# Martinsos/edlib

Measured on NVIDIA H100. Metric: GCUPS, higher is better.
Workload: dtype u32

## Files before the change

edlib_b200/csrc/eb_common.h:

```cpp
#pragma once
#include <stdint.h>

#if defined(__CUDACC__)
#define EB_HD __host__ __device__ __forceinline__
#define EB_D __device__ __forceinline__
#else
#define EB_HD inline
#define EB_D inline
#endif

namespace eb {

struct U2 { uint32_t x, y; };

constexpr int KPOS = 4;

struct Rec {
    int best;
    int cnt;
    int last;
    int rsv;
    int pos[KPOS];
};

constexpr int KPOSW = 12;
struct WinRec {
    int best, cnt, last, rsv;
    int pos[KPOSW];
};

struct Ovf {
    int rec;
    int score;
    int pos;
};

#define K1_RANGE_GAP 256
#define K1_RANGE_SPAN 1024
#define K1_RANGE_MAX 16

enum Mode : int { MODE_NW = 0, MODE_SHW = 1, MODE_HW = 2 };

struct K1Params {
    const uint8_t* tcodes;
    int n;
    const uint8_t* qcodes;
    const uint64_t* qoff;
    const int* qlen;
    const int* readList;
    const int* kInit;
    int numReads;
    int mode;
    int ncodes;
    const uint8_t* eqtab;
    int chunks;
    int chunkLen;
    int halo;
    Rec* recs;
    Ovf* ovf;
    int* ovfCount;
    int ovfCap;
    int prefixLen;
    int rangeMode;
};

struct K1WParams {
    const uint8_t* tcodes;
    const uint8_t* qcodes;
    const uint64_t* qoff;
    const int* qlen;
    const int* readList;
    const int* kInit;
    const int* winStart;
    const int* winLen;
    const int* trackFrom;
    int numReads;
    const int* countPtr;
    int checkAfter;
    int ncodes;
    const uint8_t* eqtab;
    WinRec* recs;
    Ovf* ovf;
    int* ovfCount;
    int ovfCap;
};

struct LJob {
    uint64_t qOff;
    uint64_t tOff;
    uint64_t matOff;
    int m, n;
    int kInit;
    int trackFrom;
};
struct LParams {
    const LJob* jobs;
    int numJobs;
    const uint8_t* qcodes;
    const uint8_t* tcodes;
    int ncodes;
    const uint8_t* eqtab;
    Rec* recs;
    U2* mat;
    int matStep;
};

enum WFlags : int {
    WF_QREV = 1,
    WF_TREV = 2,
    WF_SLIDE = 4,
    WF_STORE = 8,
    WF_STOPCOL = 16,
};

struct WJob {
    uint64_t qOff;
    uint64_t tOff;
    uint64_t peqOff;
    uint64_t auxOff;
    uint64_t hbufOff;
    int m, n;
    int nWp;
    int mode;
    int flags;
    int kInit;
    int dhi;
    int stopCol;
    int rec;
    int trackFrom;
};

struct WParams {
    const WJob* jobs;
    int numJobs;
    const uint8_t* qcodes;
    const uint8_t* tcodes;
    const uint32_t* peq;
// ... 250 lines not shown
```

edlib_b200/csrc/eb_core.h:

```cpp
#pragma once
#include "eb_common.h"

#if defined(__CUDA_ARCH__)
#define EB_UNROLL _Pragma("unroll")
#else
#define EB_UNROLL
#endif

namespace eb {


EB_HD uint32_t funnel_l1(uint32_t lo, uint32_t hi) {
#if defined(__CUDA_ARCH__)
    return __funnelshift_l(lo, hi, 1);
#else
    return (hi << 1) | (lo >> 31);
#endif
}

EB_HD int popcount32(uint32_t v) {
#if defined(__CUDA_ARCH__)
    return __popc(v);
#else
    return __builtin_popcount(v);
#endif
}

EB_HD int atomic_add_int(int* p, int v) {
#if defined(__CUDA_ARCH__)
    return atomicAdd(p, v);
#else
    int old = *p;
    *p = old + v;
    return old;
#endif
}

EB_HD void atomic_max_int(int* p, int v) {
#if defined(__CUDA_ARCH__)
    atomicMax(p, v);
#else
    if (v > *p) *p = v;
#endif
}

EB_HD void atomic_or_u32(uint32_t* p, uint32_t v) {
#if defined(__CUDA_ARCH__)
    atomicOr(p, v);
#else
    *p |= v;
#endif
}

template <int NW>
struct AddChain {
    static EB_HD void run(uint32_t (&S)[NW], const uint32_t (&T)[NW], const uint32_t (&P)[NW]) {
        uint32_t carry = 0;
        EB_UNROLL
        for (int w = 0; w < NW; ++w) {
            uint64_t s = (uint64_t)T[w] + P[w] + carry;
            S[w] = (uint32_t)s;
            carry = (uint32_t)(s >> 32);
        }
    }
};
#if defined(__CUDA_ARCH__)
template <>
struct AddChain<1> {
    static EB_HD void run(uint32_t (&S)[1], const uint32_t (&T)[1], const uint32_t (&P)[1]) { S[0] = T[0] + P[0]; }
};
template <>
struct AddChain<2> {
    static EB_HD void run(uint32_t (&S)[2], const uint32_t (&T)[2], const uint32_t (&P)[2]) {
        asm("add.cc.u32 %0, %2, %4;\n\taddc.u32 %1, %3, %5;"
            : "=&r"(S[0]), "=&r"(S[1]) : "r"(T[0]), "r"(T[1]), "r"(P[0]), "r"(P[1]));
    }
};
template <>
struct AddChain<3> {
    static EB_HD void run(uint32_t (&S)[3], const uint32_t (&T)[3], const uint32_t (&P)[3]) {
        asm("add.cc.u32 %0, %3, %6;\n\taddc.cc.u32 %1, %4, %7;\n\taddc.u32 %2, %5, %8;"
            : "=&r"(S[0]), "=&r"(S[1]), "=&r"(S[2])
            : "r"(T[0]), "r"(T[1]), "r"(T[2]), "r"(P[0]), "r"(P[1]), "r"(P[2]));
    }
};
template <>
struct AddChain<4> {
// ... 414 lines not shown
        }
        for (int k = 31; k >= 1; --k) {
            cur += (int)((VN0 >> k) & 1u) - (int)((VP0 >> k) & 1u);
            mn = cur < mn ? cur : mn;
        }
        return mn;
    }

    template <bool TRACK>
    EB_HD void column(int j, uint32_t sym) {
        const int gt = j + g0;
        const int wi = gt >> 5, sh = gt & 31;
        const uint32_t w0 = acc.load_word(sym, wi), w1 = acc.load_word(sym, wi + 1), w2 = acc.load_word(sym, wi + 2);
        const uint32_t Eq0 = funnel_r(w0, w1, sh), Eq1 = funnel_r(w1, w2, sh);
        uint32_t T[2] = {Eq0 & VP0, Eq1 & VP1}, P[2] = {VP0, VP1}, Sm[2];
        AddChain<2>::run(Sm, T, P);
        const uint32_t D00 = ((Sm[0] ^ VP0) | Eq0) | VN0, D01 = ((Sm[1] ^ VP1) | Eq1) | VN1;
        const uint32_t HP0 = VN0 | ~(D00 | VP0), HP1 = VN1 | ~(D01 | VP1);
        const uint32_t HN0 = VP0 & D00, HN1 = VP1 & D01;
        const uint32_t X0 = funnel_r(D00, D01, 1), X1 = D01 >> 1;
        VN0 = X0 & HP0;
        VN1 = X1 & HP1;
        VP0 = HN0 | ~(X0 | HP0);
        VP1 = HN1 | ~(X1 | HP1);
        S += 1 - (int)(HN1 >> 31);
        if (TRACK && j >= lo) {
            constexpr int CAP = (int)(sizeof(rec->pos) / sizeof(rec->pos[0]));
            const int kb = kb0 - j;
            const uint64_t M = kb >= 63 ? 0ull : (~0ull << (kb + 1));
            const int score = S - popcount32(VP0 & (uint32_t)M) - popcount32(VP1 & (uint32_t)(M >> 32)) +
                              popcount32(VN0 & (uint32_t)M) + popcount32(VN1 & (uint32_t)(M >> 32));
            if (score <= best) {
                if (score < best) {
                    best = score;
                    cnt = 0;
                }
                if (cnt < CAP) {
                    rec->pos[cnt] = ws + j;
                } else if (prm.ovfCap > 0) {
                    const int at = atomic_add_int(prm.ovfCount, 1);
                    if (at < prm.ovfCap) {
                        prm.ovf[at].rec = slot;
                        prm.ovf[at].score = score;
                        prm.ovf[at].pos = ws + j;
                    }
                }
                rec->last = ws + j;
                cnt++;
            }
        }
    }
};

template <class WAcc, class RecT>
EB_HD void k1b_sweep(const WAcc& acc, const uint8_t* tsyms, int ws, int m, int off, int c0, int lo, int hi, int t,
                     int checkAfter, int& bestIo, int& cntIo, RecT* rec, const K1WParams& prm, int slot) {
    const int dhi = hi - (m - 1) + t;
    K1Band<WAcc, RecT> b{acc, rec, 0, 0, 0, 0, 0, bestIo, cntIo, off + 64 - dhi, lo, m - 2 + dhi, ws, prm, slot};
    const int firstReal = off + 64 - (c0 + b.g0);
    const uint64_t vp64 = firstReal <= 0 ? ~0ull : (firstReal >= 64 ? 0ull : (~0ull << firstReal));
    b.VP0 = (uint32_t)vp64;
    b.VP1 = (uint32_t)(vp64 >> 32);
    const int bottomRow = c0 - dhi + 63;
    b.S = bottomRow >= 0 ? bottomRow + 1 : 0;
    int j = c0;
    for (; j <= hi && (j & 15); ++j) b.template column<true>(j, tsyms[j]);
    if (j + 15 <= hi) {
        Sym16 v = load_sym16(tsyms + j);
        bool checked = checkAfter < 0 || t == 0;
        for (; j + 15 < lo; j += 16) {
            if (!checked && j >= dhi + checkAfter) {
                checked = true;
                if (b.window_min() > t) return;
            }
            const Sym16 cur = v;
            if (j + 31 <= hi) v = load_sym16(tsyms + j + 16);
            EB_UNROLL
            for (int q = 0; q < 16; ++q) b.template column<false>(j + q, (cur.w[q >> 2] >> (8 * (q & 3))) & 255u);
        }
        for (; j + 15 <= hi; j += 16) {
            const Sym16 cur = v;
            if (j + 31 <= hi) v = load_sym16(tsyms + j + 16);
            EB_UNROLL
            for (int q = 0; q < 16; ++q) b.template column<true>(j + q, (cur.w[q >> 2] >> (8 * (q & 3))) & 255u);
        }
    }
    for (; j <= hi; ++j) b.template column<true>(j, tsyms[j]);
    bestIo = b.best;
    cntIo = b.cnt;
}

template <int NW, class WAcc>
EB_HD void k1w_thread(const K1WParams& p, int slot, WAcc& acc) {
    const int pair = p.readList[slot];
    const int m = p.qlen[pair];
    WinRec* rec = p.recs + slot;
    for (int code = 0; code < p.ncodes; ++code) {
        acc.store_word(code, 0, ~0u);
        acc.store_word(code, 1, ~0u);
        acc.store_word(code, NW + 2, 0u);
        acc.store_word(code, NW + 3, 0u);
    }
    K1View<NW, WAcc> k1acc{acc};
    k1_build_peq<NW>(k1acc, p.qcodes + p.qoff[pair], m, MODE_HW, p.ncodes, p.eqtab);
    const int ws = p.winStart[slot], tf = p.trackFrom[slot], len = p.winLen[slot];
    const int kInit = p.kInit[slot];
    const int t = kInit - 1;
    const int hi = len - 1;
    if (t >= 0 && (hi - tf) + 2 * t + 1 <= 64) {
        const int c0 = tf - (m + t) > 0 ? tf - (m + t) : 0;
        int best = kInit, cnt = 0;
        k1b_sweep(acc, p.tcodes + ws, ws, m, 32 * NW - m, c0, tf, hi, t, p.checkAfter, best, cnt, rec, p, slot);
        rec->best = best;
        rec->cnt = cnt;
        return;
    }
    K1State<NW> st;
    k1_init<NW>(st, m, kInit);
    bool hopeless = false;
    for (int j = 0; j < tf; j += 32) {
        const int cntj = tf - j < 32 ? tf - j : 32;
        k1_columns<NW, false, false>(st, k1acc, PtrSyms{p.tcodes + ws + j}, cntj, ws + j, rec, slot, nullptr, nullptr, 0);
        if (st.up - st.down - (len - (j + cntj)) >= st.best) {
            hopeless = true;
            break;
        }
    }
    if (!hopeless)
        k1_columns<NW, false, true>(st, k1acc, PtrSyms{p.tcodes + ws + tf}, len - tf, ws + tf, rec, slot, p.ovf, p.ovfCount, p.ovfCap);
    rec->best = st.best;
    rec->cnt = st.cnt;
}


EB_HD uint32_t seed_key(const uint8_t* s, int avail, int Lidx, uint32_t sigma) {
    uint32_t key = 0;
    for (int x = 0; x < Lidx; ++x) key = key * sigma + (x < avail ? (uint32_t)s[x] : 0u);
    return key;
}
EB_HD void seed_count_item(const SeedIndexParams& p, int i) {
    atomic_add_int(p.bucketStart + seed_key(p.tcodes + i, p.n - i, p.Lidx, (uint32_t)p.sigma), 1);
}
EB_HD void seed_fill_item(const SeedIndexParams& p, int i) {
    const uint32_t b = seed_key(p.tcodes + i, p.n - i, p.Lidx, (uint32_t)p.sigma);
    p.positions[p.bucketStart[b] + atomic_add_int(p.cursor + b, 1)] = i;
}

template <class F>
EB_HD int seed_windows(const SeedPlanParams& p, const int* E, int c, int m, int t, F&& f) {
    const int bandSlack = 63 - 4 * t;
    int prevHi = -1;
    int nW = 0;
    for (int i = 0; i < c;) {
        const int first = E[i];
        int last = first;
        ++i;
        if (bandSlack >= 0) {
            while (i < c && E[i] - first <= bandSlack) last = E[i++];
        } else {
            while (i < c && E[i] - last <= K1_RANGE_GAP && E[i] - first <= p.spread) last = E[i++];
        }
        int lo = first - t, hi = last + t;
        if (lo <= prevHi) lo = prevHi + 1;
        if (lo < 0) lo = 0;
        if (hi > p.n - 1) hi = p.n - 1;
        if (lo > hi) continue;
        prevHi = hi;
        int ws = lo - (m + t);
        if (ws < 0) ws = 0;
        ws &= ~15;
        f(nW, ws, lo, hi);
        ++nW;
    }
    return nW;
}
EB_HD void seed_window_store(const SeedPlanParams& p, int w, int pair, int t, int ws, int lo, int hi) {
    p.winPair[w] = pair;
    p.winK[w] = t + 1;
    p.winStart[w] = ws;
    p.winLen[w] = hi - ws + 1;
    p.winTf[w] = lo - ws;
}

struct CoopSerial {
// ... 1079 lines not shown
```

edlib_b200/csrc/eb_engine.cpp:

```cpp
#include "eb_engine_internal.h"

#include <sched.h>

namespace eb {

static int env_int(const char* name, int dflt) {
    const char* s = getenv(name);
    return (s && *s) ? atoi(s) : dflt;
}

static std::vector<int> parse_cpulist(const char* path) {
    std::vector<int> cpus;
    FILE* f = fopen(path, "r");
    if (!f) return cpus;
    char buf[4096];
    if (fgets(buf, sizeof(buf), f)) {
        for (char* tok = strtok(buf, ",\n"); tok; tok = strtok(nullptr, ",\n")) {
            int a = 0, b = 0;
            const int got = sscanf(tok, "%d-%d", &a, &b);
            if (got == 1) b = a;
            if (got >= 1)
                for (int c = a; c <= b && c < 4096; ++c) cpus.push_back(c);
        }
    }
// ... 6 lines not shown
    if (cpus.empty()) return;
    cpu_set_t allowed, want;
    CPU_ZERO(&allowed);
    CPU_ZERO(&want);
    if (sched_getaffinity(0, sizeof(allowed), &allowed) != 0) return;
    int n = 0;
    for (int c : cpus)
        if (c < CPU_SETSIZE && CPU_ISSET(c, &allowed)) {
            CPU_SET(c, &want);
            ++n;
        }
    if (n > 0) sched_setaffinity(0, sizeof(want), &want);
}

void host_parallel_ranges(size_t n, size_t grain, const std::function<void(size_t, size_t)>& fn) {
    parallel_ranges(n, grain, [&](size_t lo, size_t hi) { fn(lo, hi); });
}

Engine::Engine(Backend* be) : be_(be) {
    if (env_int("EDLIB_B200_NUMA", 1) == 0) return;
    const int node = be->numa_node();
    if (node < 0) return;
    char path[128];
    snprintf(path, sizeof(path), "/sys/devices/system/node/node%d/cpulist", node);
    std::vector<int> cpus = parse_cpulist(path);
    if (!cpus.empty() && HostPool::worker_cpus().empty()) HostPool::worker_cpus() = cpus;
}

EngineTunables::EngineTunables() {
    k1MinGroup = env_int("EDLIB_B200_K1_MIN_GROUP", k1MinGroup);
    k1MinChunk = env_int("EDLIB_B200_K1_MIN_CHUNK", k1MinChunk);
    ovfCap = env_int("EDLIB_B200_OVF_CAP", ovfCap);
    filterK0 = env_int("EDLIB_B200_FILTER_K0", filterK0);
    filterK1 = env_int("EDLIB_B200_FILTER_K1", filterK1);
    packParallelBytes = (size_t)env_int("EDLIB_B200_PACK_PARALLEL_KB", (int)(packParallelBytes >> 10)) << 10;
    filterSeedK = env_int("EDLIB_B200_FILTER_SEED_K", filterSeedK);
    filterSeedBucket = env_int("EDLIB_B200_FILTER_SEED_BUCKET", filterSeedBucket);
    filterSeedSlack = env_int("EDLIB_B200_FILTER_SEED_SLACK", filterSeedSlack);
    filterMinLevelReads = env_int("EDLIB_B200_FILTER_MIN_LEVEL_READS", filterMinLevelReads);
    tinySweepReads = env_int("EDLIB_B200_TINY_SWEEP_READS", tinySweepReads);
    filterSeedLevels = std::min(SEED_LEVELS, env_int("EDLIB_B200_FILTER_SEED_LEVELS", filterSeedLevels));
    filterMaxWindows = env_int("EDLIB_B200_FILTER_MAX_WINDOWS", filterMaxWindows);
    filterMinLen = env_int("EDLIB_B200_FILTER_MIN_LEN", filterMinLen);
    filterSpread = env_int("EDLIB_B200_FILTER_SPREAD", filterSpread);
    filterMinTarget = env_int("EDLIB_B200_FILTER_MIN_TARGET", filterMinTarget);
    filterSkipRepeats = env_int("EDLIB_B200_FILTER_SKIP_REPEATS", filterSkipRepeats);
    bandKernel = env_int("EDLIB_B200_BAND_KERNEL", bandKernel);
    collapseEqualities = env_int("EDLIB_B200_COLLAPSE_EQUALITIES", collapseEqualities);
    directUpload = env_int("EDLIB_B200_DIRECT_UPLOAD", directUpload);
    streamSlices = std::max(1, env_int("EDLIB_B200_STREAM_SLICES", streamSlices));
    directMinBytes = (size_t)env_int("EDLIB_B200_DIRECT_MIN_KB", (int)(directMinBytes >> 10)) << 10;
    deviceStage = env_int("EDLIB_B200_DEVICE_STAGE", deviceStage);
    windowCheckAfter = env_int("EDLIB_B200_WINDOW_CHECK", windowCheckAfter);
    longHwMinTarget = env_int("EDLIB_B200_LONG_HW_MIN_TARGET", longHwMinTarget);
    longSeedMaxK = env_int("EDLIB_B200_LONG_SEED_MAX_K", longSeedMaxK);
    devSliceReads = std::max(64, env_int("EDLIB_B200_SLICE_READS", devSliceReads));
    streamMinPairs = env_int("EDLIB_B200_STREAM_MIN_PAIRS", streamMinPairs);
    const int sliceMb = env_int("EDLIB_B200_SLICE_MB", 0);
    if (sliceMb > 0) sliceBytes = (size_t)sliceMb << 20;
    if (sliceMb > 0) pathSliceBytes = (size_t)sliceMb << 20;
}

static int code_map(const uint32_t (&present)[8], uint8_t (&map)[256], int other) {
    int ncodes = 0;
    for (int b = 0; b < 256; ++b) ncodes += (present[b >> 5] >> (b & 31)) & 1u;
    int next = 0;
    for (int b = 0; b < 256; ++b) {
        if (present[b >> 5] >> (b & 31) & 1u) map[b] = (uint8_t)next++;
        else map[b] = (uint8_t)(other < 0 ? 0 : std::min(other, 255));
    }
    return ncodes;
}

static int encode_target(Backend* be, uint8_t* raw, int n, TargetCodes& tc) {
    std::vector<MaskItem> items;
    for (int s0 = 0; s0 < n; s0 += 65536) items.push_back(MaskItem{(uint64_t)s0, std::min(65536, n - s0), 0});
    DevBuf<MaskItem> dItems(be, items.size());
    dItems.upload(items.data(), items.size());
    tc.dMask.alloc(be, 8);
    be->zero(tc.dMask.p, 8 * sizeof(uint32_t));
    MaskParams mp;
    memset(&mp, 0, sizeof(mp));
    mp.raw = raw;
    mp.items = dItems.p;
    mp.numItems = (int)items.size();
    mp.masks = tc.dMask.p;
    mp.unionSet = -1;
    be->launch_mask(mp);
    uint32_t present[8];
    be->d2h(present, tc.dMask.p, sizeof(present));
    int distinct = 0;
    for (int b = 0; b < 256; ++b) distinct += (present[b >> 5] >> (b & 31)) & 1u;
    uint8_t map[256];
    code_map(present, map, distinct);
    tc.dMap.alloc(be, 256);
    tc.dMap.upload(map, 256);
    EncodeParams ep{raw, (uint64_t)round_up((size_t)n, 16), tc.dMap.p};
    be->launch_encode(ep);
    tc.ncodes = distinct >= 256 ? 256 : std::max(1, std::min(distinct, 255));
    return tc.ncodes;
}

Prepared* Engine::take_prepared(const BatchInput& in) {
    if (!spare_) spare_ = new Prepared();
    Prepared* p = spare_;
    p->bind(be_);
// ... 1040 lines not shown
```

edlib_b200/csrc/eb_engine.h:

```cpp
#pragma once
#include <stddef.h>
#include <stdint.h>

#include <map>
#include <string>
#include <utility>
#include <vector>

#include "../../include/edlib.h"
#include "eb_common.h"

namespace eb {

struct Backend {
    virtual ~Backend() {}
    virtual void* alloc(size_t bytes) = 0;
    virtual void free(void* p) = 0;
    virtual void* alloc_host(size_t bytes) = 0;
    virtual void free_host(void* p) = 0;
    virtual bool host_pinned(const void* , size_t ) { return false; }
    virtual void h2d(void* dst, const void* src, size_t bytes) = 0;
    virtual void d2h(void* dst, const void* src, size_t bytes) = 0;
    virtual void zero(void* dst, size_t bytes) = 0;
    virtual void d2d(void* dst, const void* src, size_t bytes) = 0;
// ... 12 lines not shown
    virtual int sm_count() = 0;
    virtual void k1_shape(int nw32, int ncodes, int numReads, int* blockThreads, int* residentCtas) = 0;
    virtual void launch_mask(const MaskParams& p) = 0;
    virtual void launch_alpha_len(const uint32_t* masks, const int* qset, const int* tset, int numPairs, int* out) = 0;
    virtual void launch_encode(const EncodeParams& p) = 0;
    virtual void launch_k1(const K1Params& p, int nw32) = 0;
    virtual void launch_k1t(const K1Params& p, int nw32) = 0;
    virtual void launch_k1w(const K1WParams& p, int nw32) = 0;
    virtual void launch_lane(const LParams& p, int nw32, int mode, bool reversed, bool store) = 0;
    virtual void launch_peq(const PeqParams& p) = 0;
    virtual void launch_w(const WParams& p, int R) = 0;
    virtual int band_max_blocks(int ncodes) = 0;
    virtual void launch_band(const WParams& p, int NB, int ncodes) = 0;
    virtual void launch_traceback(const TbParams& p) = 0;
    virtual void launch_res(const ResParams& p) = 0;
    virtual void launch_split(const SplitParams& p) = 0;
    virtual void launch_seed_count(const SeedIndexParams& p) = 0;
    virtual void launch_scan(int* data, int count) = 0;
    virtual void launch_seed_fill(const SeedIndexParams& p) = 0;
    virtual void launch_seed_plan(const SeedPlanParams& p) = 0;
    virtual void launch_win_reduce(const WinReduceParams& p) = 0;
    virtual void launch_fin_count(const FinParams& p) = 0;
    virtual void launch_fin_fill(const FinParams& p) = 0;
    virtual void launch_qalpha(const QAlphaParams& p) = 0;
    virtual void reset_timing() = 0;
    virtual double kernel_ms(const char* nameOrNull) = 0;
    virtual int launches() = 0;
    virtual std::string kernel_report() = 0;
};

struct BatchInput {
    const char* const* queries;
    const int* queryLengths;
    const char* const* targets;
    const int* targetLengths;
    int numPairs;
    EdlibAlignConfig config;
    bool strands = false;
};

struct EngineTunables {
    int k1MinGroup = 32;
    int k1MinChunk = 1024;
    int ovfCap = 1 << 20;
    size_t sliceBytes = 1ull << 30;
    size_t pathSliceBytes = 8ull << 30;
    size_t packParallelBytes = 32u << 20;
    int deviceStage = 1;
    int devSliceReads = 1 << 20;
    int streamSlices = 8;
    int streamMinPairs = 32768;
    int longHwMinTarget = 65536;
    int longSeedMaxK = 1024;
    int windowCheckAfter = 48;
    int filterSeedK = 20;
    int filterSeedBucket = 128;
    int filterSeedLevels = 4;
    int tinySweepReads = 8;
    int filterMinLevelReads = 64;
    int filterSeedSlack = 4;
    int filterK1 = 8;
    int filterK0 = 16;
    int filterMinLen = 96;
    int filterSpread = 1024;
    int filterMaxWindows = 32;
    int filterMinTarget = 65536;
    size_t directMinBytes = 1u << 20;
    int directUpload = 1;
    int collapseEqualities = 1;
    int bandKernel = 1;
    int filterSkipRepeats = 1;
    EngineTunables();
};

struct EngineStats {
    double kernelMs = 0;
    double k1Ms = 0;
    int launches = 0;
    long long h2dBytes = 0, d2hBytes = 0;
    long long k1Cells = 0;
    long long wCells = 0;
    long long filterDecided = 0, filterFallback = 0;
    long long filterWindows = 0;
    std::string kernelReport;
};

struct EngineScratch {
    std::vector<int> best, cnt, posLen, posPool;
    std::vector<long long> posStart;
    int seedWindowsPerRead[SEED_LEVELS] = {0, 0, 0, 0};
    std::vector<int> targetTable;
};

class Prepared;
struct TargetHandle;

class Engine {
public:
    explicit Engine(Backend* be);
    ~Engine();
    int align_batch(const BatchInput& in, EdlibAlignResult* results, unsigned char* strands = nullptr);
    void strands_of(const Prepared* p, unsigned char* strands) const;

    Prepared* prepare(const BatchInput& in);
    void compute(Prepared* p);
    void materialize(Prepared* p, EdlibAlignResult* results, const std::vector<int>* list = nullptr);
    void release(Prepared* p);
// ... 25 lines not shown
```

edlib_b200/csrc/eb_kernels.cu:

```cuda
#include <cuda_runtime.h>
#include <ctype.h>
#include <stdio.h>
#include <sys/syscall.h>
#include <unistd.h>
#include <stdlib.h>
#include <string.h>

#include <algorithm>
#include <mutex>
#include <stdexcept>
#include <string>
#include <vector>

#include "eb_core.h"
#include "eb_dispatch.h"
#include "eb_engine.h"

namespace eb {

#if defined(__CUDA_ARCH__)
#define EB_DEV(expr, fallback) expr
#else
#define EB_DEV(expr, fallback) fallback
#endif
// ... 213 lines not shown
    EB_D void store(int code, int word, uint32_t bits) { w[code * NW + word] = bits; }
    EB_D void or_word(int code, int word, uint32_t bits) { w[code * NW + word] |= bits; }
    EB_D void load(uint32_t code, uint32_t (&Eq)[NW]) const {
#pragma unroll
        for (int i = 0; i < NW; ++i) Eq[i] = w[code * NW + i];
    }
};
template <int NW>
__global__ void __launch_bounds__(32) k1t_kernel(const K1Params p) {
    extern __shared__ __align__(16) unsigned char smem[];
    WarpPeqAcc<NW> acc{reinterpret_cast<uint32_t*>(smem)};
    const int slot = blockIdx.y;
    const int chunk = blockIdx.x * 32 + threadIdx.x;
    if (threadIdx.x == 0) {
        const int pair = p.readList[slot];
        k1_build_peq<NW>(acc, p.qcodes + p.qoff[pair], p.qlen[pair], p.mode, p.ncodes, p.eqtab);
    }
    __syncwarp();
    if (chunk < p.chunks) k1_thread<NW, WarpPeqAcc<NW>, false>(p, slot, chunk, acc);
}

template <int THREADS, int WORDS>
struct SmemWordAcc {
    uint32_t base;
    static constexpr uint32_t wordStride = 4u * THREADS, codeStride = wordStride * WORDS;
    EB_D void store_word(int code, int w, uint32_t bits) {
        asm volatile("st.shared.u32 [%0], %1;" ::"r"(base + (uint32_t)code * codeStride + (uint32_t)w * wordStride), "r"(bits) : "memory");
    }
    EB_D void or_word(int code, int w, uint32_t bits) {
        const uint32_t addr = base + (uint32_t)code * codeStride + (uint32_t)w * wordStride;
        uint32_t v;
        asm volatile("ld.shared.u32 %0, [%1];" : "=r"(v) : "r"(addr) : "memory");
        asm volatile("st.shared.u32 [%0], %1;" ::"r"(addr), "r"(v | bits) : "memory");
    }
    EB_D uint32_t load_word(uint32_t code, int w) const {
        uint32_t v;
        asm volatile("ld.shared.u32 %0, [%1];" : "=r"(v) : "r"(base + code * codeStride + (uint32_t)w * wordStride));
        return v;
    }
};

template <int NW, int THREADS>
__global__ void __launch_bounds__(THREADS) k1w_kernel(const K1WParams p) {
    extern __shared__ __align__(128) unsigned char smem[];
    const int slot = blockIdx.x * THREADS + threadIdx.x;
    int numJobs = p.numReads;
    if (p.countPtr) numJobs = min(numJobs, *p.countPtr);
    if (slot >= numJobs) return;
    SmemWordAcc<THREADS, NW + 4> acc;
    acc.base = smem_u32(smem) + 4u * threadIdx.x;
    k1w_thread<NW>(p, slot, acc);
}

template <int NW, int MODE, bool REV, bool STORE>
__global__ void lane_kernel(const LParams p) {
    extern __shared__ __align__(128) unsigned char smem[];
    const int job = blockIdx.x * blockDim.x + threadIdx.x;
    if (job >= p.numJobs) return;
    SmemPeqAcc<NW> acc;
    acc.codeStride = (uint32_t)blockDim.x * (16u + 4u * SmemPeqAcc<NW>::NWB);
    acc.a0 = smem_u32(smem) + 16u * threadIdx.x;
    acc.b0 = smem_u32(smem) + 16u * blockDim.x + 4u * SmemPeqAcc<NW>::NWB * threadIdx.x;
    lane_job<NW, MODE, REV, STORE>(p, job, acc);
}

constexpr int W_WARPS = 4;

template <int R>
__global__ void __launch_bounds__(W_WARPS * 32) w_kernel(const WParams p) {
    const int job = blockIdx.x * W_WARPS + (threadIdx.x >> 5);
    if (job >= p.numJobs) return;
    w_dispatch<DevWarp, R>(p, job);
}

template <int THREADS, int SLOTS>
struct SmemBandAcc {
    uint32_t base, cur;
    static constexpr uint32_t wordStride = 4u * THREADS, codeStride = wordStride * SLOTS;
    EB_D void set(int code, int slot, uint32_t bits) {
        asm volatile("st.shared.u32 [%0], %1;" ::"r"(base + (uint32_t)code * codeStride + (uint32_t)slot * wordStride), "r"(bits) : "memory");
    }
    EB_D uint32_t get(int code, int slot) const {
        uint32_t v;
        asm volatile("ld.shared.u32 %0, [%1];" : "=r"(v) : "r"(base + (uint32_t)code * codeStride + (uint32_t)slot * wordStride) : "memory");
        return v;
    }
    EB_D void origin(int slot) { cur = base + (uint32_t)slot * wordStride; }
    EB_D uint32_t code_off(uint32_t sym) const { return sym * codeStride; }
    EB_D uint32_t load(uint32_t codeOff, int w) const {
        uint32_t v;
        asm volatile("ld.shared.u32 %0, [%1];" : "=r"(v) : "r"(cur + codeOff + (uint32_t)w * wordStride) : "memory");
        return v;
    }
};
constexpr int BAND_THREADS = 128;
template <int NB>
__global__ void __launch_bounds__(BAND_THREADS) band_kernel(const WParams p, int ncodes) {
    extern __shared__ __align__(128) unsigned char smem[];
    const int job = blockIdx.x * BAND_THREADS + threadIdx.x;
    if (job >= p.numJobs) return;
    SmemBandAcc<BAND_THREADS, 4 * NB + BAND_SLACK> acc;
    acc.base = smem_u32(smem) + 4u * threadIdx.x;
    acc.cur = acc.base;
    band_job<NB>(p, job, acc, ncodes);
}

// ... 465 lines not shown
        size_t smem;
        k1_block(nw, ncodes, numReads, &block, &smem);
        if (shapeCache.empty()) shapeCache.assign(4 * 9 * 1024, 0);
        const int blockClass = block >= 256 ? 3 : block >= 128 ? 2 : block >= 64 ? 1 : 0;
        const int key = (blockClass * 9 + nw) * 1024 + (ncodes < 1024 ? ncodes : 1023);
        if (ncodes < 1023 && shapeCache[key]) {
            *blockThreads = shapeCache[key] & 0xfff;
            *residentCtas = shapeCache[key] >> 12;
            return;
        }
        if (smem > (size_t)maxSmemOptin || (size_t)ncodes * 4 * (nw + 4) * 32 > (size_t)maxSmemOptin) {
            *blockThreads = block;
            *residentCtas = 0;
            return;
        }
        int perSm = 1;
        with_nw(nw, [&](auto w) { perSm = k1_occupancy<decltype(w)::value>(block, smem); });
        *blockThreads = block;
        *residentCtas = perSm * sms;
        if (ncodes < 1023) shapeCache[key] = block | ((perSm * sms) << 12);
    }
    void launch_k1t(const K1Params& p, int nw) override {
        if (p.rangeMode || p.prefixLen > 0) throw std::runtime_error("k1t: plain sweeps only");
        const size_t smem = (size_t)p.ncodes * nw * sizeof(uint32_t);
        const dim3 grid((unsigned)((p.chunks + 31) / 32), (unsigned)p.numReads);
        with_nw(nw, [&](auto w) { launch("k1", k1t_kernel<decltype(w)::value>, grid, 32, smem, p); });
    }
    void launch_k1(const K1Params& p, int nw) override {
        int block;
        size_t smem;
        k1_block(nw, p.ncodes, p.numReads, &block, &smem);
        if (smem > (size_t)maxSmemOptin) throw std::runtime_error("K1: alphabet too large for shared memory");
        const dim3 grid((p.numReads + block - 1) / block, p.chunks);
        if (p.rangeMode) {
            const char* bad = "range mode needs the 1- or 2-word HW kernel";
            if (p.mode != MODE_HW) throw std::runtime_error(bad);
            with_one_of<1, 2>(nw, bad, [&](auto w) { launch("k1_prefix", k1_kernel<decltype(w)::value, MODE_HW, true>, grid, block, smem, p); });
            return;
        }
        with_nw(nw, [&](auto w) {
            with_mode(p.mode, [&](auto m) { launch("k1", k1_kernel<decltype(w)::value, decltype(m)::value>, grid, block, smem, p); });
        });
    }
    void launch_k1w(const K1WParams& p, int nw) override {
        int block = 128;
        const size_t perThread = (size_t)p.ncodes * 4 * (nw + 4);
        while (block > 32 && perThread * block > 96 * 1024) block >>= 1;
        const size_t smem = perThread * block;
        if (smem > (size_t)maxSmemOptin) throw std::runtime_error("K1W: alphabet too large for shared memory");
        with_nw(nw, [&](auto w) {
            with_one_of<128, 64, 32>(block, "bad K1W CTA size", [&](auto threads) {
                constexpr int THREADS = decltype(threads)::value;
                launch("k1w", k1w_kernel<decltype(w)::value, THREADS>, (p.numReads + THREADS - 1) / THREADS, THREADS, smem, p);
            });
        });
    }
    void launch_lane(const LParams& p, int nw, int mode, bool rev, bool store) override {
        int block = 128;
        const size_t perThread = (size_t)p.ncodes * (16 + 4 * (nw > 4 ? nw - 4 : 0));
        while (block > 32 && perThread * block > 96 * 1024) block >>= 1;
        const size_t smem = perThread * block;
        if (smem > (size_t)maxSmemOptin) throw std::runtime_error("lane kernel: alphabet too large for shared memory");
        with_nw(nw, [&](auto w) {
            with_lane_class(mode, rev, store, [&](auto c) {
                using C = decltype(c);
                launch("lane", lane_kernel<decltype(w)::value, C::MODE, C::REV, C::STORE>, (p.numJobs + block - 1) / block, block, smem, p);
            });
        });
    }
    void launch_res(const ResParams& p) override {
        if (p.numItems <= 0) return;
        launch("res", res_kernel, (p.numItems + 255) / 256, 256, 0, p);
    }
    void launch_peq(const PeqParams& p) override {
        launch("peq", peq_kernel, (p.numJobs + W_WARPS - 1) / W_WARPS, W_WARPS * 32, 0, p);
    }
    void launch_w(const WParams& p, int R) override {
        with_r(R, [&](auto r) { launch("w", w_kernel<decltype(r)::value>, (p.numJobs + W_WARPS - 1) / W_WARPS, W_WARPS * 32, 0, p); });
    }
    static size_t band_smem(int NB, int ncodes) { return (size_t)ncodes * (4 * NB + BAND_SLACK) * 4 * BAND_THREADS; }
    int band_max_blocks(int ncodes) override {
        int nb = 0;
        while (nb < 8 && band_smem(nb + 1, ncodes) <= (size_t)110 * 1024) ++nb;
        return nb;
    }
    void launch_band(const WParams& p, int NB, int ncodes) override {
        with_nb(NB, [&](auto nb) {
            launch("band", band_kernel<decltype(nb)::value>, (p.numJobs + BAND_THREADS - 1) / BAND_THREADS, BAND_THREADS, band_smem(NB, ncodes), p,
                   ncodes);
        });
    }
    void launch_seed_count(const SeedIndexParams& p) override { launch("seed_count", seed_count_kernel, (p.numPos + 255) / 256, 256, 0, p); }
    void launch_seed_fill(const SeedIndexParams& p) override { launch("seed_fill", seed_fill_kernel, (p.numPos + 255) / 256, 256, 0, p); }
    void launch_scan(int* data, int count) override {
        if (count <= 0) {
            zero(data, sizeof(int));
            return;
        }
        const int numTiles = (count + SCAN_TILE - 1) / SCAN_TILE;
        int* tileSums = static_cast<int*>(alloc((size_t)numTiles * sizeof(int)));
        launch("scan", scan_tile_sums_kernel, numTiles, SCAN_THREADS, 0, data, count, tileSums);
        launch("scan", scan_top_kernel, 1, 1024, 0, tileSums, numTiles, data + count);
        launch("scan", scan_apply_kernel, numTiles, SCAN_THREADS, 0, data, count, tileSums);
        free(tileSums);
    }
    template <int CAP, int THREADS, int GW>
// ... 95 lines not shown
```

edlib_b200/csrc/eb_pass_lane.cpp:

```cpp
#include "eb_engine_internal.h"

namespace eb {

bool build_seed_index(Backend* be, const EngineTunables& tun, SeedIndex& sx, const uint8_t* tcodes, int n, int ncodes) {
    sx.n = n;
    sx.ok = false;
    const int sigma = std::max(2, ncodes);
    int L0 = 4;
    double v = std::pow((double)sigma, 4);
    while (v < (double)tun.filterSeedSlack * (double)n && L0 < 32) {
        v *= sigma;
        ++L0;
    }
    if (n < 4 * L0) return false;
    const int step = (sigma * sigma <= 32) ? 2 : 1;
    for (int level = 0; level < SEED_LEVELS; ++level) {
        const int L = level < 3 ? L0 - step * level : L0 - step * 2 - (level - 2);
        const bool useful = L >= 4 && (level == 0 || (double)n / std::pow((double)sigma, L) <= 128.0);
        sx.Ls[level] = useful ? L : 0;
    }
    int Lidx = 1;
    long long keys = sigma;
    const long long maxKeys = std::min<long long>(std::max<long long>(2LL * n, 4096), 1LL << 28);
    while (Lidx < 16 && keys * sigma <= maxKeys) {
// ... 53 lines not shown
    sp.Lidx = sx.Lidx;
    sp.sigma = sx.sigma;
    sp.numKeys = sx.numKeys;
    sp.bucketStart = sx.bucketStart.p;
    sp.positions = sx.positions.p;
    sp.maxBucket = std::min(tun.filterSeedBucket << (1 + 3 * level), 8192);
    sp.level = level;
    sp.spread = tun.filterSpread;
    return sp;
}

int Pass::plan_windows(SeedPlanParams sp, WinJobs& jobs, int cap, bool hostCount) {
    for (;;) {
        jobs.alloc(be, cap);
        sp.winPair = jobs.pair.p;
        sp.winK = jobs.k.p;
        sp.winStart = jobs.start.p;
        sp.winLen = jobs.len.p;
        sp.winTf = jobs.tf.p;
        sp.winCap = cap;
        sp.winCount = jobs.count;
        be->launch_seed_plan(sp);
        if (!hostCount) return -1;
        int V = 0;
        be->d2h(&V, jobs.count, sizeof(int));
        stats.d2hBytes += 4;
        if (V <= cap) return V;
        cap = V;
        be->zero(jobs.count, sizeof(int));
    }
}

void Pass::sweep_windows(const Target& tg, int nw, const WinJobs& jobs, int numJobs, const WinRecords& out) {
    K1WParams wp;
    memset(&wp, 0, sizeof(wp));
    wp.tcodes = p->dSeq.p + tg.off;
    wp.qcodes = p->dSeq.p;
    wp.qoff = p->dQoff.p;
    wp.qlen = p->dQlen.p;
    wp.readList = jobs.pair.p;
    wp.kInit = jobs.k.p;
    wp.winStart = jobs.start.p;
    wp.winLen = jobs.len.p;
    wp.trackFrom = jobs.tf.p;
    wp.numReads = numJobs < 0 ? jobs.cap : numJobs;
    wp.countPtr = numJobs < 0 ? jobs.count : nullptr;
    wp.checkAfter = tun.windowCheckAfter;
    wp.ncodes = p->ncodes;
    wp.eqtab = p->hasEq ? p->dEqtab.p : nullptr;
    wp.recs = out.recs;
    wp.ovf = out.ovf;
    wp.ovfCount = out.ovfCount;
    wp.ovfCap = out.ovfCap;
    be->launch_k1w(wp, nw);
}

void Pass::reduce_windows(WinReduceParams rp, const SeedPlan* plan, int numReads, const WinRecords& wr, Rec* out, int* extra,
                          int* extraCount, int extraCap) {
    rp.plan = plan;
    rp.winRecs = wr.recs;
    rp.numReads = numReads;
    rp.out = out;
    rp.extra = extra;
    rp.extraCount = extraCount;
    rp.extraCap = extraCap;
    rp.ovf = wr.ovf;
    rp.ovfCount = wr.ovfCount;
    rp.ovfCap = wr.ovfCap;
    be->launch_win_reduce(rp);
}

void Pass::lane_geometry(const LaneGroup& c, int g, int nwL, int& chunks, int& chunkLen, bool perChunkRecs) {
    const int n = c.n;
    int blockThreads = 256, residentCtas = 1;
    be->k1_shape(nwL, p->ncodes, g, &blockThreads, &residentCtas);
    chunks = 1;
    chunkLen = (int)round_up((size_t)n, 16);
    if (mode != MODE_HW) return;
    const int minChunk = std::max(tun.k1MinChunk, (g <= 32 ? 2 : 8) * 64 * nwL);
    long long maxChunks = std::max<long long>(1, n / minChunk);
    if (perChunkRecs) maxChunks = std::min<long long>(maxChunks, std::max<long long>(64, (2LL << 20) / std::max(g, 1)));
    maxChunks = std::min<long long>(maxChunks, 4096);
    const long long tiles = ceil_div(g, blockThreads);
    long long best = 1;
    double bestScore = -1;
    for (long long c = 1; c <= maxChunks; ++c) {
        const double waves = (double)(tiles * c) / residentCtas;
        const double eff = waves / (double)((tiles * c + residentCtas - 1) / residentCtas);
        const double len = (double)n / (double)c;
        const double score = eff * (len / (len + 64.0 * nwL));
        if (score > bestScore + 0.002) {
            bestScore = score;
            best = c;
        }
    }
    chunkLen = (int)round_up((size_t)ceil_div(n, (int)best), 16);
    chunks = ceil_div(n, chunkLen);
}

void Pass::lane_sweep(LaneGroup& c, const std::vector<int>& sub, const std::vector<int>& subK, int nwL, int chunks, int chunkLen,
                int cap, int prefixLen, int rangeMode, std::vector<Rec>& outRecs, std::vector<Ovf>& outOvf) {
    const std::vector<int>& list = c.list;
    const Target& tg = c.tg;
    const int n = c.n;
    const int g = (int)sub.size();
    std::vector<int> rl(g);
    for (int s = 0; s < g; ++s) rl[s] = list[sub[s]];
// ... 669 lines not shown
```

Measured before the change: 95.38 million.

## Compact surviving k1w band threads into a resume kernel after early-exit check

At the early-exit check in the banded window sweep, threads that survive save their band state and Peq to a compacted buffer via a warp-coalesced atomic, then exit. A second kernel resumes only the survivors, so warps there stay fully occupied instead of idling on lanes that already exited. The check point moves earlier (from 48 to 32 columns) and resume capacity defaults to half the windows. The cost is extra global memory traffic for the saved state, extra allocations and one more kernel launch per call.

```diff
diff --git a/edlib_b200/csrc/eb_common.h b/edlib_b200/csrc/eb_common.h
--- a/edlib_b200/csrc/eb_common.h
+++ b/edlib_b200/csrc/eb_common.h
@@ -64,6 +64,11 @@
     int rangeMode;
 };
 
+struct BandResume {
+    uint32_t VP0, VP1, VN0, VN1;
+    int S, j, slot, pad;
+};
+
 struct K1WParams {
     const uint8_t* tcodes;
     const uint8_t* qcodes;
@@ -83,6 +88,10 @@
     Ovf* ovf;
     int* ovfCount;
     int ovfCap;
+    BandResume* resume;
+    uint32_t* resumePeq;
+    int* resumeCount;
+    int resumeCap;
 };
 
 struct LJob {
diff --git a/edlib_b200/csrc/eb_core.h b/edlib_b200/csrc/eb_core.h
--- a/edlib_b200/csrc/eb_core.h
+++ b/edlib_b200/csrc/eb_core.h
@@ -33,6 +33,19 @@
     int old = *p;
     *p = old + v;
     return old;
+#endif
+}
+
+EB_HD int atomic_inc_coalesced(int* p) {
+#if defined(__CUDA_ARCH__)
+    const unsigned mask = __activemask();
+    const int lane = (int)(threadIdx.x & 31u), leader = __ffs(mask) - 1;
+    int base = 0;
+    if (lane == leader) base = atomicAdd(p, __popc(mask));
+    base = __shfl_sync(mask, base, leader);
+    return base + __popc(mask & ((1u << lane) - 1u));
+#else
+    return atomic_add_int(p, 1);
 #endif
 }
 
@@ -553,26 +566,41 @@
     }
 };
 
+
+constexpr int K1B_NO_CHECK = 0x7fffffff;
+
 template <class WAcc, class RecT>
-EB_HD void k1b_sweep(const WAcc& acc, const uint8_t* tsyms, int ws, int m, int off, int c0, int lo, int hi, int t,
-                     int checkAfter, int& bestIo, int& cntIo, RecT* rec, const K1WParams& prm, int slot) {
+EB_HD K1Band<WAcc, RecT> k1b_band(const WAcc& acc, RecT* rec, const K1WParams& prm, int slot, int ws, int m, int off, int lo,
+                                  int hi, int t) {
     const int dhi = hi - (m - 1) + t;
-    K1Band<WAcc, RecT> b{acc, rec, 0, 0, 0, 0, 0, bestIo, cntIo, off + 64 - dhi, lo, m - 2 + dhi, ws, prm, slot};
-    const int firstReal = off + 64 - (c0 + b.g0);
-    const uint64_t vp64 = firstReal <= 0 ? ~0ull : (firstReal >= 64 ? 0ull : (~0ull << firstReal));
-    b.VP0 = (uint32_t)vp64;
-    b.VP1 = (uint32_t)(vp64 >> 32);
-    const int bottomRow = c0 - dhi + 63;
-    b.S = bottomRow >= 0 ? bottomRow + 1 : 0;
-    int j = c0;
+    return K1Band<WAcc, RecT>{acc, rec, 0, 0, 0, 0, 0, t + 1, 0, off + 64 - dhi, lo, m - 2 + dhi, ws, prm, slot};
+}
+
+template <class WAcc, class RecT>
+EB_HD int k1b_columns(K1Band<WAcc, RecT>& b, const uint8_t* tsyms, int j, int hi, int t, int checkAt) {
+    const int lo = b.lo;
     for (; j <= hi && (j & 15); ++j) b.template column<true>(j, tsyms[j]);
     if (j + 15 <= hi) {
         Sym16 v = load_sym16(tsyms + j);
-        bool checked = checkAfter < 0 || t == 0;
         for (; j + 15 < lo; j += 16) {
-            if (!checked && j >= dhi + checkAfter) {
-                checked = true;
-                if (b.window_min() > t) return;
+            if (j >= checkAt) {
+                checkAt = K1B_NO_CHECK;
+                if (b.window_min() > t) return -1;
+                if (b.prm.resumeCap > 0) {
+                    const int at = atomic_inc_coalesced(b.prm.resumeCount);
+                    if (at < b.prm.resumeCap) {
+                        BandResume& r = b.prm.resume[at];
+                        r.VP0 = b.VP0;
+                        r.VP1 = b.VP1;
+                        r.VN0 = b.VN0;
+                        r.VN1 = b.VN1;
+                        r.S = b.S;
+                        r.j = j;
+                        r.slot = b.slot;
+                        r.pad = 0;
+                        return at;
+                    }
+                }
             }
             const Sym16 cur = v;
             if (j + 31 <= hi) v = load_sym16(tsyms + j + 16);
@@ -587,21 +615,28 @@
         }
     }
     for (; j <= hi; ++j) b.template column<true>(j, tsyms[j]);
-    bestIo = b.best;
-    cntIo = b.cnt;
-}
+    return -1;
+}
+
+template <int NW, class WAcc>
+EB_HD void k1w_profile_frame(const K1WParams& p, WAcc& acc) {
+    for (int code = 0; code < p.ncodes; ++code) {
+        acc.store_word(code, 0, ~0u);
+        acc.store_word(code, 1, ~0u);
+        acc.store_word(code, NW + 2, 0u);
+        acc.store_word(code, NW + 3, 0u);
+    }
+}
+
+template <int NW, class WAcc>
+EB_HD void k1w_resume_thread(const K1WParams& p, int i, WAcc& acc);
 
 template <int NW, class WAcc>
 EB_HD void k1w_thread(const K1WParams& p, int slot, WAcc& acc) {
     const int pair = p.readList[slot];
     const int m = p.qlen[pair];
     WinRec* rec = p.recs + slot;
-    for (int code = 0; code < p.ncodes; ++code) {
-        acc.store_word(code, 0, ~0u);
-        acc.store_word(code, 1, ~0u);
-        acc.store_word(code, NW + 2, 0u);
-        acc.store_word(code, NW + 3, 0u);
-    }
+    k1w_profile_frame<NW>(p, acc);
     K1View<NW, WAcc> k1acc{acc};
     k1_build_peq<NW>(k1acc, p.qcodes + p.qoff[pair], m, MODE_HW, p.ncodes, p.eqtab);
     const int ws = p.winStart[slot], tf = p.trackFrom[slot], len = p.winLen[slot];
@@ -610,10 +645,31 @@
     const int hi = len - 1;
     if (t >= 0 && (hi - tf) + 2 * t + 1 <= 64) {
         const int c0 = tf - (m + t) > 0 ? tf - (m + t) : 0;
-        int best = kInit, cnt = 0;
-        k1b_sweep(acc, p.tcodes + ws, ws, m, 32 * NW - m, c0, tf, hi, t, p.checkAfter, best, cnt, rec, p, slot);
-        rec->best = best;
-        rec->cnt = cnt;
+        const int off = 32 * NW - m;
+        K1Band<WAcc, WinRec> b = k1b_band(acc, rec, p, slot, ws, m, off, tf, hi, t);
+        const int dhi = hi - (m - 1) + t;
+        const int firstReal = off + 64 - (c0 + b.g0);
+        const uint64_t vp64 = firstReal <= 0 ? ~0ull : (firstReal >= 64 ? 0ull : (~0ull << firstReal));
+        b.VP0 = (uint32_t)vp64;
+        b.VP1 = (uint32_t)(vp64 >> 32);
+        const int bottomRow = c0 - dhi + 63;
+        b.S = bottomRow >= 0 ? bottomRow + 1 : 0;
+        const int checkAt = p.checkAfter < 0 || t == 0 ? K1B_NO_CHECK : dhi + p.checkAfter;
+        const int at = k1b_columns(b, p.tcodes + ws, c0, hi, t, checkAt);
+        if (at >= 0) {
+            for (int code = 0; code < p.ncodes; ++code) {
+                EB_UNROLL
+                for (int w = 0; w < NW; ++w) p.resumePeq[(size_t)(code * NW + w) * p.resumeCap + at] = acc.load_word(code, w + 2);
+            }
+#if !defined(__CUDA_ARCH__)
+            for (int code = 0; code < p.ncodes; ++code)
+                for (int w = 0; w < NW + 4; ++w) acc.store_word(code, w, 0xdeadbeefu);
+            k1w_resume_thread<NW>(p, at, acc);
+#endif
+            return;
+        }
+        rec->best = b.best;
+        rec->cnt = b.cnt;
         return;
     }
     K1State<NW> st;
@@ -631,6 +687,31 @@
         k1_columns<NW, false, true>(st, k1acc, PtrSyms{p.tcodes + ws + tf}, len - tf, ws + tf, rec, slot, p.ovf, p.ovfCount, p.ovfCap);
     rec->best = st.best;
     rec->cnt = st.cnt;
+}
+
+template <int NW, class WAcc>
+EB_HD void k1w_resume_thread(const K1WParams& p, int i, WAcc& acc) {
+    const BandResume r = p.resume[i];
+    const int slot = r.slot;
+    const int m = p.qlen[p.readList[slot]];
+    k1w_profile_frame<NW>(p, acc);
+    for (int code = 0; code < p.ncodes; ++code) {
+        EB_UNROLL
+        for (int w = 0; w < NW; ++w) acc.store_word(code, w + 2, p.resumePeq[(size_t)(code * NW + w) * p.resumeCap + i]);
+    }
+    WinRec* rec = p.recs + slot;
+    const int ws = p.winStart[slot];
+    const int t = p.kInit[slot] - 1;
+    const int hi = p.winLen[slot] - 1;
+    K1Band<WAcc, WinRec> b = k1b_band(acc, rec, p, slot, ws, m, 32 * NW - m, p.trackFrom[slot], hi, t);
+    b.VP0 = r.VP0;
+    b.VP1 = r.VP1;
+    b.VN0 = r.VN0;
+    b.VN1 = r.VN1;
+    b.S = r.S;
+    k1b_columns(b, p.tcodes + ws, r.j, hi, t, K1B_NO_CHECK);
+    rec->best = b.best;
+    rec->cnt = b.cnt;
 }
 
 
diff --git a/edlib_b200/csrc/eb_engine.cpp b/edlib_b200/csrc/eb_engine.cpp
--- a/edlib_b200/csrc/eb_engine.cpp
+++ b/edlib_b200/csrc/eb_engine.cpp
@@ -82,6 +82,7 @@
     directMinBytes = (size_t)env_int("EDLIB_B200_DIRECT_MIN_KB", (int)(directMinBytes >> 10)) << 10;
     deviceStage = env_int("EDLIB_B200_DEVICE_STAGE", deviceStage);
     windowCheckAfter = env_int("EDLIB_B200_WINDOW_CHECK", windowCheckAfter);
+    windowResumePct = std::min(100, std::max(0, env_int("EDLIB_B200_WINDOW_RESUME_PCT", windowResumePct)));
     longHwMinTarget = env_int("EDLIB_B200_LONG_HW_MIN_TARGET", longHwMinTarget);
     longSeedMaxK = env_int("EDLIB_B200_LONG_SEED_MAX_K", longSeedMaxK);
     devSliceReads = std::max(64, env_int("EDLIB_B200_SLICE_READS", devSliceReads));
diff --git a/edlib_b200/csrc/eb_engine.h b/edlib_b200/csrc/eb_engine.h
--- a/edlib_b200/csrc/eb_engine.h
+++ b/edlib_b200/csrc/eb_engine.h
@@ -88,7 +88,8 @@
     int streamMinPairs = 32768;
     int longHwMinTarget = 65536;
     int longSeedMaxK = 1024;
-    int windowCheckAfter = 48;
+    int windowCheckAfter = 32;
+    int windowResumePct = 50;
     int filterSeedK = 20;
     int filterSeedBucket = 128;
     int filterSeedLevels = 4;
diff --git a/edlib_b200/csrc/eb_kernels.cu b/edlib_b200/csrc/eb_kernels.cu
--- a/edlib_b200/csrc/eb_kernels.cu
+++ b/edlib_b200/csrc/eb_kernels.cu
@@ -289,6 +289,16 @@
     k1w_thread<NW>(p, slot, acc);
 }
 
+template <int NW, int THREADS>
+__global__ void __launch_bounds__(THREADS) k1w_resume_kernel(const K1WParams p) {
+    extern __shared__ __align__(128) unsigned char smem[];
+    const int i = blockIdx.x * THREADS + threadIdx.x;
+    if (i >= min(*p.resumeCount, p.resumeCap)) return;
+    SmemWordAcc<THREADS, NW + 4> acc;
+    acc.base = smem_u32(smem) + 4u * threadIdx.x;
+    k1w_resume_thread<NW>(p, i, acc);
+}
+
 template <int NW, int MODE, bool REV, bool STORE>
 __global__ void lane_kernel(const LParams p) {
     extern __shared__ __align__(128) unsigned char smem[];
@@ -860,6 +870,9 @@
             with_one_of<128, 64, 32>(block, "bad K1W CTA size", [&](auto threads) {
                 constexpr int THREADS = decltype(threads)::value;
                 launch("k1w", k1w_kernel<decltype(w)::value, THREADS>, (p.numReads + THREADS - 1) / THREADS, THREADS, smem, p);
+                if (p.resumeCap > 0)
+                    launch("k1w_resume", k1w_resume_kernel<decltype(w)::value, THREADS>, (p.resumeCap + THREADS - 1) / THREADS,
+                           THREADS, smem, p);
             });
         });
     }
diff --git a/edlib_b200/csrc/eb_pass_lane.cpp b/edlib_b200/csrc/eb_pass_lane.cpp
--- a/edlib_b200/csrc/eb_pass_lane.cpp
+++ b/edlib_b200/csrc/eb_pass_lane.cpp
@@ -129,7 +129,30 @@
     wp.ovf = out.ovf;
     wp.ovfCount = out.ovfCount;
     wp.ovfCap = out.ovfCap;
+    DevBuf<BandResume> resume;
+    DevBuf<uint32_t> resumePeq;
+    DevBuf<int> resumeCount;
+    if (tun.windowResumePct > 0 && wp.numReads > 0 && p->ncodes * nw <= 64) {
+        wp.resumeCap = (int)(((long long)wp.numReads * tun.windowResumePct + 99) / 100);
+        resume.alloc(be, (size_t)wp.resumeCap);
+        resumePeq.alloc(be, (size_t)wp.resumeCap * p->ncodes * nw);
+        resumeCount.alloc(be, 1);
+        be->zero(resumeCount.p, sizeof(int));
+        wp.resume = resume.p;
+        wp.resumePeq = resumePeq.p;
+        wp.resumeCount = resumeCount.p;
+    }
     be->launch_k1w(wp, nw);
+    if (trace.on && wp.resumeCap > 0) {
+        int survivors = 0, windows = wp.numReads;
+        resumeCount.download(&survivors, 1);
+        if (wp.countPtr) {
+            be->d2h(&windows, wp.countPtr, sizeof(int));
+            windows = std::min(windows, wp.numReads);
+        }
+        fprintf(stderr, "[edlib_b200] k1w: %d windows, %d past the early exit, %d of them resumed\n", windows, survivors,
+                std::min(survivors, wp.resumeCap));
+    }
 }
 
 void Pass::reduce_windows(WinReduceParams rp, const SeedPlan* plan, int numReads, const WinRecords& wr, Rec* out, int* extra,
```

New measurement: 99.51 million (median of 6 runs). 1.04x the previous value.
